# lovesh/bulletproofs-r1cs-gadgets

Hardware: AMD Instinct MI355X
Metric: R1CS proofs/sec (Poseidon VSMT-4 depth-32) (higher is better)
Workload: dtype int32; 1 GPU; gadget_vsmt_4 sparse-Merkle depth-32 membership (Poseidon 4:1 inverse S-box, 148 rounds); distinct_inputs_steps=9, batch_per_gpu=1024, global_batch=1024, n_multipliers=18656, padded_n=32768, constraints=43330, proof_bytes=1377, proofs_per_device_job=4096, device_jobs=3, jobs_in_flight=2, warmup_steps_run=5, ipa_unfold_rounds=4, table_window_bits=11, table_windows=23, table_format=1, table_bytes=197767468800

## Files before the change

bulletproofs-r1cs-gadgets_amd/csrc/api_prove.hpp:

```cpp
#pragma once
#include "ipa.hpp"
#include "host_chain.hpp"
struct bpr1cs_job {
    const bpr1cs_gens* g = nullptr;
    dev_stream_t st{}, st2{}, st3{}, st4{};
    std::vector<void*> deferred;
    PhaseTimer pt;
    MsmStats msm;
    uint32_t B = 0, m = 0;
    size_t plen = 0;
    uint8_t* h_proofs = nullptr;
    uint8_t* h_comms = nullptr;
    int* h_err = nullptr;
    uint32_t* h_chk = nullptr;
    strobe* h_tr = nullptr;
    bool counted = false;
    int slot = -1;
    IpaIO::TailKeep tail;
    dev_event_t ev_in{}, ev_rng{}, ev_wit{}, ev_done{}, ev_tail{};
    uint8_t* h_in = nullptr;
    size_t h_in_bytes = 0;
    uint8_t* h_V = nullptr;
    uint64_t* h_raw = nullptr;
    size_t h_raw_bytes = 0;
    strobe* h_tr0 = nullptr;
    bool host_chain = false;
    uint32_t Bh = 0;
    dev_event_t ev_head{};
};
struct HostStage {
    std::mutex mu;
    std::multimap<size_t, void*> cache;
    std::map<void*, size_t> live;
};
inline HostStage& host_stage() {
    static HostStage* h = new HostStage();
    return *h;
}
static void* host_stage_alloc(size_t n) {
    if (n == 0) n = 1;
#if defined(BPR1CS_HOSTSIM)
    return malloc(n);
#else
    HostStage& hs = host_stage();
    std::lock_guard<std::mutex> lk(hs.mu);
    auto it = hs.cache.lower_bound(n);
    void* p = nullptr;
    size_t sz = n;
    if (it != hs.cache.end() && it->first <= 2 * n + 4096) { p = it->second; sz = it->first; hs.cache.erase(it); }
    else HIPCHK(hipHostMalloc(&p, n, hipHostMallocDefault));
    hs.live[p] = sz;
    return p;
#endif
}
static void host_stage_free(void* p) {
#if defined(BPR1CS_HOSTSIM)
    free(p);
#else
    if (!p) return;
    HostStage& hs = host_stage();
    std::lock_guard<std::mutex> lk(hs.mu);
    auto it = hs.live.find(p);
    if (it == hs.live.end()) return;
    hs.cache.insert({it->second, p});
    hs.live.erase(it);
#endif
}
static bool dbg_jobs() {
    static const bool on = getenv("BPR1CS_DEBUG_JOBS") != nullptr;
    return on;
}
static double dbg_ms() {
    static const auto t0 = std::chrono::steady_clock::now();
    return std::chrono::duration<double, std::milli>(std::chrono::steady_clock::now() - t0).count();
}
#define DBG_JOB(...) do { if (dbg_jobs()) { fprintf(stderr, "bpr1cs[%9.2f ms] ", dbg_ms()); fprintf(stderr, __VA_ARGS__); fputc('\n', stderr); } } while (0)
static void host_wipe(void* p, size_t n) { explicit_bzero(p, n); }
static void job_wait(bpr1cs_job* job) {
    if (!job) return;
    if (job->ev_done) (void)dev_event_sync(job->ev_done);
#if !defined(BPR1CS_HOSTSIM)
    else if (job->st) (void)hipStreamSynchronize(job->st);
    if (job->st2) (void)hipStreamSynchronize(job->st2);
    if (job->st3) (void)hipStreamSynchronize(job->st3);
#endif
}
static void job_release(bpr1cs_job* job) {
    if (!job) return;
    job_wait(job);
#if !defined(BPR1CS_HOSTSIM)
    for (auto e : job->pt.ev) (void)hipEventDestroy(e);
    job->pt.ev.clear();
#endif
    dev_event_t* evs[6] = {&job->ev_in, &job->ev_rng, &job->ev_wit, &job->ev_done, &job->ev_tail, &job->ev_head};
    for (auto e : evs) dev_event_destroy(e);
    for (void* p : job->deferred) dev_free_now(p);
    job->deferred.clear();
    if (job->h_raw) host_wipe(job->h_raw, job->h_raw_bytes);
    if (job->h_in) host_wipe(job->h_in, job->h_in_bytes);
    if (job->h_tr0 && job->Bh) host_wipe(job->h_tr0, (size_t)job->Bh * sizeof(strobe));
    host_stage_free(job->h_in);
    host_stage_free(job->h_raw);
    host_stage_free(job->h_V);
    host_stage_free(job->h_tr0);
    host_stage_free(job->h_proofs);
    host_stage_free(job->h_comms);
    host_stage_free(job->h_err);
    host_stage_free(job->h_chk);
    host_stage_free(job->h_tr);
    if (job->counted) job->g->in_flight--;
    if (job->slot >= 0) job->g->busy_slots.fetch_and(~(1u << job->slot));
    delete job;
}

static TabCfg merged_tab_cfg(const bpr1cs_gens* g, uint32_t T3) {
#if defined(BPR1CS_HOSTSIM)
    const char* force = getenv("BPR1CS_TEST_NARROW_MERGED");
// ... 21 lines not shown
static void enqueue_witness_check(const bpr1cs_circuit* c, const sc* W, const sc* v_m, uint32_t* res, uint32_t B, dev_stream_t s) {
    {
        std::lock_guard<std::mutex> lk(c->mt_mu);
        if (!c->rows_uploaded) {
            ArenaScope persistent(nullptr);
            upload(c->row_off, c->h_row_off, s);
            upload(c->row_slot, c->h_row_slot, s);
            upload(c->row_coeff, c->h_row_coeff, s);
            upload(c->row_chunk, c->h_row_chunk, s);
            c->rows_uploaded = true;
        }
    }
    const uint32_t Bpad = (B + 63u) & ~63u;
    launch(B, K_check_init{res}, s);
    launch((uint64_t)((c->n + CHECK_GATES - 1) / CHECK_GATES) * Bpad, K_check_gates{W, res, B, Bpad, c->n}, s);
    const uint32_t nchunks = (uint32_t)c->h_row_chunk.size() - 1, per_launch = 0xffffffffu / Bpad;
    for (uint32_t c0 = 0; c0 < nchunks; c0 += per_launch)
        launch((uint64_t)std::min(per_launch, nchunks - c0) * Bpad,
               K_check_rows{c->row_chunk.p, c->row_off.p, c->row_slot.p, c->row_coeff.p, W, v_m, res, B, Bpad, 3 * c->n, c->m, c0}, s);
}

static int prove_job_begin(const bpr1cs_gens* g, const bpr1cs_circuit* c, const strobe* init, size_t n_init, bool want_tr,
                           const uint8_t* values, const uint8_t* v_blindings, const uint8_t* rng_seeds,
                           const uint8_t* wires, size_t batch, bpr1cs_job** job_out, const uint8_t* ext_draws = nullptr, int auto_share = 0) {
    if (!g || !c || !init || (!rng_seeds && !ext_draws) || !job_out || batch == 0 || (n_init != 1 && n_init != batch)) return BPR1CS_ERR_INVALID_ARGUMENT;
    if (ext_draws && n_init != batch) return BPR1CS_ERR_INVALID_ARGUMENT;
    if (c->m && (!values || !v_blindings)) return BPR1CS_ERR_INVALID_ARGUMENT;
    if (!have_device()) return BPR1CS_ERR_NO_DEVICE;
    if (g->cap < c->N) return BPR1CS_ERR_INVALID_GENERATORS_LENGTH;
    if (!wires && !c->has_program) return BPR1CS_ERR_MISSING_ASSIGNMENT;
    if (batch > (1u << 20) || ((uint64_t)4 * c->N + 3ull * c->n + c->m + 64) * batch > 0xffffffffull) return BPR1CS_ERR_INVALID_ARGUMENT;
    if (c->m && (!host_scalars_canonical(values, batch * c->m) || !host_scalars_canonical(v_blindings, batch * c->m))) return BPR1CS_ERR_INVALID_ARGUMENT;
    if (wires && !host_scalars_canonical(wires, batch * 3 * (size_t)c->n)) return BPR1CS_ERR_INVALID_ARGUMENT;
    bpr1cs_job* job = nullptr;
    struct Scope {
        std::vector<void*>* prev;
        explicit Scope(bpr1cs_job* j) : prev(dev_deferred_frees()) { dev_deferred_frees() = &j->deferred; }
        ~Scope() { dev_deferred_frees() = prev; }
    };
    uint32_t slot = 0;
    for (;;) {
        uint32_t busy = g->busy_slots.load();
        if ((busy & 3u) == 3u) return BPR1CS_ERR_INVALID_ARGUMENT;
        slot = (busy & 1u) ? 1u : 0u;
        if (g->busy_slots.compare_exchange_weak(busy, busy | (1u << slot))) break;
    }
    try {
// ... 60 lines not shown
        HIPCHK(hipGetLastError());
    } else
#endif
    launch((uint64_t)m * B, K_commit_v{g->tab.p, g->tc, v_raw.p, vbl_raw.p, Vcomp.p, B, m}, sl);
    DevBuf<strobe> tr(B);
    const bool shared = g->opts.shared_back.load() != 0;
    DevBuf<sc> blind((size_t)8 * B), W;
    DevBuf<uint64_t> rng_raw;
    const uint32_t draws = 2 * n + 7;
    const int o_hc = g->opts.host_chain.load();
    const bool ext = ext_draws != nullptr;
    const bool host_chain = !ext && (o_hc < 0 ? B <= 4u * host_cpu_budget() : B <= (uint32_t)o_hc);
    job->host_chain = host_chain;
    uint32_t Bh = 0;
    const unsigned chain_workers = host_cpu_budget() - 1;
#if !defined(BPR1CS_HOSTSIM)
    if (!ext && !host_chain && chain_workers > 0) {
        const int o_share = g->opts.host_chain_share.load();
        const int share = o_share >= 0 ? o_share : std::max(0, std::min(100, auto_share));
        Bh = (uint32_t)(((uint64_t)B * (uint32_t)share + 50) / 100);
    }
#endif
    job->Bh = Bh;
    {
        ArenaScope sh(shared ? &g->shared_front : &g->front[slot], shared);
        W.alloc((size_t)5 * n * B + 1);
        rng_raw.alloc((size_t)(draws + (host_chain || ext ? 1 : 0)) * B * 8);
    }
    sc* sL = W.p + (size_t)3 * n * B;
    sc* sR = W.p + (size_t)4 * n * B;
    pt.mark(sl);
    dev_event_create(&job->ev_in);
    dev_event_create(&job->ev_rng);
    dev_event_record(job->ev_in, sl);
    DevBuf<int> rng_err(1);
    dev_zero(rng_err.p, sizeof(int), sl);
    DevBuf<strobe> rng;
    HostChains chains;
    if (ext) {
        job->h_raw_bytes = (size_t)(draws + 1) * B * 64;
        job->h_raw = (uint64_t*)host_stage_alloc(job->h_raw_bytes);
        memcpy(job->h_raw, ext_draws, job->h_raw_bytes);
        dev_d2d(tr.p, d_init.p, (size_t)B * sizeof(strobe), sl);
        if (shared) dev_stream_wait(sl, g->rng_free_ev);
        dev_h2d_async(rng_raw.p, job->h_raw, job->h_raw_bytes, sl);
        if (shared) dev_stream_wait(sl, g->w_free_ev);
        launch((uint64_t)(draws + 1) * B, K_rng_reduce{rng_raw.p, blind.p, sL, sR, B, n, 1u}, sl);
        dev_zero(rng_raw.p, rng_raw.bytes(), sl);
        if (shared) dev_event_record(g->rng_free_ev, sl);
        dev_event_record(job->ev_rng, sl);
    } else if (host_chain) {
        job->h_V = (uint8_t*)host_stage_alloc((size_t)B * m * 32);
        if (m) dev_d2h_async(job->h_V, Vcomp.p, (size_t)B * m * 32, sl);
        job->h_raw_bytes = (size_t)(draws + 1) * B * 64;
        job->h_raw = (uint64_t*)host_stage_alloc(job->h_raw_bytes);
        job->h_tr0 = (strobe*)host_stage_alloc((size_t)B * sizeof(strobe));
    } else {
#if defined(BPR1CS_HOSTSIM)
        launch_transcript(B, K_transcript_init{d_init.p, init_stride, Vcomp.p, vbl_raw.p, d_seeds.p, tr.p, blind.p, sL, sR, nullptr, B, m, n}, sl);
#else
        rng.alloc(B);
        launch_transcript(B, K_transcript_init{d_init.p, init_stride, Vcomp.p, vbl_raw.p, d_seeds.p, tr.p, blind.p, sL, sR, rng.p, B, m, n}, sl);
        if (Bh) {
            job->h_tr0 = (strobe*)host_stage_alloc((size_t)Bh * sizeof(strobe));
            dev_d2h_async(job->h_tr0, rng.p, (size_t)Bh * sizeof(strobe), sl);
            dev_event_create(&job->ev_head);
            dev_event_record(job->ev_head, sl);
        }
        if (shared) dev_stream_wait(sl, g->rng_free_ev);
        if (Bh < B) {
            hipLaunchKernelGGL(k_rng_stream, dim3((B - Bh + 1) / 2), dim3(64), 0, sl, rng.p + Bh, rng_raw.p + (size_t)draws * Bh * 8, rng_err.p, B - Bh, draws);
            HIPCHK(hipGetLastError());
        }
        if (!Bh) {
            if (shared) dev_stream_wait(sl, g->w_free_ev);
            launch((uint64_t)draws * B, K_rng_reduce{rng_raw.p, blind.p, sL, sR, B, n, 0u}, sl);
            dev_zero(rng_raw.p, rng_raw.bytes(), sl);
            dev_zero(rng.p, rng.bytes(), sl);
            if (shared) dev_event_record(g->rng_free_ev, sl);
        }
#endif
        if (!Bh) dev_event_record(job->ev_rng, sl);
    }

    if (host_chain) {
        dev_sync(sl);
        DBG_JOB("begin: %u host chain(s) start", B);
        chains.start(init, n_init, job->h_V, v_blindings, rng_seeds, B, m, n, job->h_tr0, job->h_raw);
        if ((uint64_t)B * (draws + 1) <= 4096) chains.wait();
    }

    DevBuf<sc> px;
    struct { uint32_t* p; } chk{nullptr};
    if (o_check) {
        DevBuf<uint32_t>& blk = g->check_res[slot];
        if (blk.n < (size_t)4 * B) { ArenaScope persistent(nullptr); blk.alloc((size_t)4 * B); }
        chk.p = blk.p;
    }
    if (wires) {
        const dev_stream_t sw = job->st3;
        DevBuf<sc> raw((size_t)3 * n * B);
        static_assert(sizeof(sc) == 32, "a canonical scalar's 32 little-endian bytes are an sc as they are");
        if (raw.bytes()) dev_h2d(raw.p, wires, raw.bytes(), sw);
        if (shared) dev_stream_wait(sw, g->w_free_ev);
        launch((uint64_t)3 * n * B, K_load_wires_pm{raw.p, W.p, B, 3 * n}, sw);
// ... 15 lines not shown
            kw.px = px.p; kw.pzf = pzf.p; kw.px_stride = c->px_stride;
        }
#if defined(BPR1CS_HOSTSIM)
        (void)o_team;
        launch(B, kw, st);
        if (o_check) enqueue_witness_check(c, W.p, v_m.p, chk.p, B, st);
#else
        int T = o_team;
        if (c->n_perms && (uint32_t)T < c->macro_width + 2) T = 16;
        kw.prio = 2;
        uint32_t blocks = (uint32_t)(((uint64_t)B * T + 63) / 64);
        dev_stream_wait(job->st3, job->ev_in);
        if (shared) dev_stream_wait(job->st3, g->w_free_ev);
        if (T == 4) hipLaunchKernelGGL(HIP_KERNEL_NAME(k_witness_team<4>), dim3(blocks), dim3(64), 0, job->st3, kw);
        else if (T == 8) hipLaunchKernelGGL(HIP_KERNEL_NAME(k_witness_team<8>), dim3(blocks), dim3(64), 0, job->st3, kw);
        else hipLaunchKernelGGL(HIP_KERNEL_NAME(k_witness_team<16>), dim3(blocks), dim3(64), 0, job->st3, kw);
        HIPCHK(hipGetLastError());
        if (o_check) enqueue_witness_check(c, W.p, v_m.p, chk.p, B, job->st3);
        dev_event_create(&job->ev_wit);
        dev_event_record(job->ev_wit, job->st3);
        dev_stream_wait(st, job->ev_wit);
#endif
    }
    auto finish_split = [&]() {
        if (!Bh) return;
        const uint32_t Dc = 256, R = 4;
        const dev_stream_t su = job->st3;
        if (!dev_event_sync(job->ev_head)) throw DevError{BPR1CS_ERR_DEVICE};
        job->h_raw_bytes = (size_t)R * Dc * Bh * 64;
        job->h_raw = (uint64_t*)host_stage_alloc(job->h_raw_bytes);
        if (shared) dev_stream_wait(su, g->rng_free_ev);
        dev_event_t ev_slot[R] = {};
        for (uint32_t r = 0; r < R; r++) dev_event_create(&ev_slot[r]);
        struct Events { dev_event_t* e; uint32_t n; ~Events() { for (uint32_t r = 0; r < n; r++) dev_event_destroy(&e[r]); } } evs_guard{ev_slot, R};
        uint64_t* raw_h = rng_raw.p;
        DBG_JOB("begin: %u host chain(s) of %u streamed (%.4f us per permutation and worker)", Bh, B, host_chain_us_per_perm());
        double busy_us = 0;
        const bool ok = host_chains_stream(job->h_tr0, Bh, draws, Dc, R, job->h_raw, chain_workers,
            [&](uint32_t, uint32_t slot, uint32_t d0, uint32_t nd) {
                dev_h2d_async(raw_h + (size_t)d0 * Bh * 8, job->h_raw + (size_t)slot * Dc * Bh * 8, (size_t)nd * Bh * 64, su);
                dev_event_record(ev_slot[slot], su);
            },
            [&](uint32_t slot) { if (!dev_event_sync(ev_slot[slot])) throw DevError{BPR1CS_ERR_DEVICE}; }, chain8_select(), &busy_us);
        if (ok && busy_us > 0) host_chain_rate_cell().store(busy_us / ((double)Bh * draws));
        host_wipe(job->h_tr0, (size_t)Bh * sizeof(strobe));
        if (!ok) throw DevError{BPR1CS_ERR_INVALID_ARGUMENT};
        DBG_JOB("begin: host chain(s) hashed");
        dev_event_record(job->ev_head, su);
        dev_stream_wait(sl, job->ev_head);
        if (shared) dev_stream_wait(sl, g->w_free_ev);
        launch((uint64_t)draws * Bh, K_rng_reduce{raw_h, blind.p, sL, sR, B, n, 0u, Bh, 0u}, sl);
        if (Bh < B) launch((uint64_t)draws * (B - Bh), K_rng_reduce{raw_h + (size_t)draws * Bh * 8, blind.p, sL, sR, B, n, 0u, B - Bh, Bh}, sl);
        dev_zero(rng_raw.p, rng_raw.bytes(), sl);
        dev_zero(rng.p, rng.bytes(), sl);
        if (shared) dev_event_record(g->rng_free_ev, sl);
        dev_event_record(job->ev_rng, sl);
    };
    auto finish_host_chains = [&]() {
        finish_split();
        if (!host_chain) return;
        chains.wait();
        DBG_JOB("begin: host chain(s) done");
        dev_h2d_async(tr.p, job->h_tr0, (size_t)B * sizeof(strobe), sl);
        if (shared) dev_stream_wait(sl, g->rng_free_ev);
        dev_h2d_async(rng_raw.p, job->h_raw, job->h_raw_bytes, sl);
        if (shared) dev_stream_wait(sl, g->w_free_ev);
        launch((uint64_t)(draws + 1) * B, K_rng_reduce{rng_raw.p, blind.p, sL, sR, B, n, 1u}, sl);
        dev_zero(rng_raw.p, rng_raw.bytes(), sl);
        if (shared) dev_event_record(g->rng_free_ev, sl);
        dev_event_record(job->ev_rng, sl);
    };
    DBG_JOB("begin: front enqueued");
    DevBuf<uint8_t> AOS((size_t)3 * B * 32);
    DevBuf<sc> chal((size_t)CH_COUNT * B), txs((size_t)3 * B), uk((size_t)(lgN ? lgN : 1) * 2 * B);
    DevBuf<uint8_t> Tc((size_t)5 * B * 32), LR((size_t)(lgN ? lgN : 1) * 2 * B * 32);
    const size_t plen = bpr1cs_proof_len(c);
    job->plen = plen;
    DevBuf<uint8_t> d_out((size_t)B * plen);
    ArenaScope back_arena(shared ? &g->arena : &g->front[slot], shared);
    DevBuf<ge> partial, partialO;
    MsmPlan plan;
    {
// ... 28 lines not shown
                }
                mtab = mt->tab.p;
                mtc = mt->tc;
                ones_pt = mt->ones_pt.p;
            }
            const uint32_t nr = (uint32_t)c->h_rest.size();
            MsmSeg rG{aL, nr, 1, 1, 0, baseG, 1, c->rest.p, 0}, rH{aR, nr, 1, 1, 0, baseH, 1, c->rest.p, 0};
            MsmSeg mG{aL, T3, 1, 1, 0, 0, 1, c->trip.p, 1}, mH{aR, T3, 1, 1, 0, T3, 1, c->trip.p, 1};
            MsmPlan plan2;
            MsmSeg oRest{aO, nr, 1, 1, 0, baseG, MSM_MONT, c->rest.p, 0}, oOnes{aO, 2 * T3, 1, 1, 0, baseG, MSM_MINUS_ONE, c->ones.p, 0};
            MsmReq rq[4] = {{rG, rH, &partial, &plan, nullptr}, {mG, mH, &partial2, &plan2, mtab, 0, &mtc}, {oRest, none, &partialO, &planO, nullptr},
                            {oOnes, none, &partialO1, &planO1, nullptr, 256}};
            run_msm_multi(g, rq, 4, B, st, stats);
            finI.partial = partial.p;
            finI.nchunks = plan.nchunks;
            finI.partial_b = partial2.p;
            finI.nchunks_b = plan2.nchunks;
        } else {
            MsmReq rq[2] = {{seg(aL, baseG), seg(aR, baseH), &partial, &plan, nullptr}, {seg(aO, baseG), none, &partialO, &planO, nullptr}};
            run_msm_multi(g, rq, 2, B, st, stats, nullptr, ct);
            finI.partial = partial.p;
            finI.nchunks = plan.nchunks;
        }
        finish_host_chains();
        dev_stream_wait(st, job->ev_rng);
        pt.mark(st);
        if (ct) {
            DevBuf<ge> pbI, pbO, pbS;
            MsmPlan plI, plO, plS;
            auto bl = [&](uint32_t k) { return MsmSeg{blind.p + (size_t)k * B, 1, 1, 1, 0, 1, MSM_MONT}; };
            MsmReq rq[4] = {{seg(sL, baseG), seg(sR, baseH), &partialS, &planS, nullptr}, {bl(0), none, &pbI, &plI, nullptr},
                            {bl(1), none, &pbO, &plO, nullptr}, {bl(2), none, &pbS, &plS, nullptr}};
            run_msm_multi(g, rq, 4, B, st, stats, nullptr, true);
            finI.extra = nullptr; finI.partial_b = pbI.p; finI.nchunks_b = plI.nchunks;
            K_msm_finish finO{g->tab.p, g->tc, partialO.p, nullptr, nullptr, AOS.p + 1 * (size_t)B * 32, B, planO.nchunks, 1};
            finO.partial_b = pbO.p; finO.nchunks_b = plO.nchunks;
            K_msm_finish finS{g->tab.p, g->tc, partialS.p, nullptr, nullptr, AOS.p + 2 * (size_t)B * 32, B, planS.nchunks, 1};
            finS.partial_b = pbS.p; finS.nchunks_b = plS.nchunks;
            launch(B, finI, st);
            launch(B, finO, st);
            launch(B, finS, st);
        } else {
        K_msm_finish finO{g->tab.p, g->tc, partialO.p, blind.p + 1 * (size_t)B, nullptr, AOS.p + 1 * (size_t)B * 32, B, planO.nchunks, 1};
        if (ones_pt) { finO.shared_pt = ones_pt; finO.partial_b = partialO1.p; finO.nchunks_b = planO1.nchunks; }
        if (B <= SMALL_JOB_PROOFS) {
            run_msm(g, seg(sL, baseG), seg(sR, baseH), B, partialS, planS, st, stats);
            launch_finish_triple(finI, finO, K_msm_finish{g->tab.p, g->tc, partialS.p, blind.p + 2 * (size_t)B, nullptr, AOS.p + 2 * (size_t)B * 32, B, planS.nchunks, 1}, B, st);
        } else {
            launch_finish(finI, B, st);
            launch_finish(finO, B, st);
            run_msm(g, seg(sL, baseG), seg(sR, baseH), B, partial, plan, st, stats);
            launch_finish(K_msm_finish{g->tab.p, g->tc, partial.p, blind.p + 2 * (size_t)B, nullptr, AOS.p + 2 * (size_t)B * 32, B, plan.nchunks, 1}, B, st);
        }
        }
    }
    pt.mark(st);

    launch_transcript(B, K_transcript_A{tr.p, AOS.p, chal.p, B}, st);
    uint32_t maxe = std::max<uint32_t>(N, c->q + 1);
    uint32_t H = (maxe >> 8) + 1;
    DevBuf<sc> plo((size_t)3 * 256 * B), phi((size_t)3 * H * B);
    launch_pow_tables(K_pow_tables{chal.p, plo.p, phi.p, B, H}, B, st);
    const uint32_t r_eff = std::min<uint32_t>((uint32_t)o_unfold, lgN);
    const bool fvec = g->opts.factor_vectors.load() == 1;
    const uint32_t nfl = c->h_slot_chunk[3 * n + m];
    auto al = [](size_t x) { return (x + 255) & ~(size_t)255; };
    const size_t w_bytes = al(((size_t)(3 * n + m) * B + 1) * sizeof(sc)), p_bytes = al((size_t)(nfl ? nfl : 1) * B * sizeof(sc)),
                 v_bytes = al((size_t)N * B * sizeof(sc));
    const size_t vt_count = r_eff < lgN ? (size_t)VB_MULT * 4 * ((N >> r_eff) / 2 ? (N >> r_eff) / 2 : 1) * B : 0;
    const bool need_s = r_eff > 0 || (!fvec && lgN > 0);
    const size_t others = w_bytes + p_bytes + (fvec ? 2 * v_bytes : 0) + (need_s ? 2 * v_bytes : 0);
    DevBuf<uint8_t> shared_blk(std::max(others, vt_count * sizeof(ge_cached)));
    sc* wvec_p = (sc*)shared_blk.p;
    sc* fpart_p = (sc*)(shared_blk.p + w_bytes);
    uint8_t* nxt = shared_blk.p + w_bytes + p_bytes;
// ... 233 lines not shown
    J = std::min(J, grid_max);
    const size_t m = c->m, plen = bpr1cs_proof_len(c), wn = 3 * (size_t)c->n;
    struct Pending { bpr1cs_job* job; size_t first; };
    std::vector<Pending> fl;
    int rc = BPR1CS_OK;
    size_t ended = 0;
    auto finish_oldest = [&]() {
        Pending p = fl.front();
        fl.erase(fl.begin());
        ended += p.job->B;
        int e = prove_job_end(p.job, proofs_out + p.first * plen, commitments_out ? commitments_out + p.first * m * 32 : nullptr,
                              tr_out ? tr_out + p.first : nullptr, &acc);
        if (e != BPR1CS_OK && rc == BPR1CS_OK) rc = e;
    };
    size_t done = 0;
    bool retried = false;
    double prior_ms_per_proof = 0;
    {
        std::lock_guard<std::mutex> lk(c->mt_mu);
        auto it = c->mt.find(g);
        if (it != c->mt.end()) prior_ms_per_proof = it->second->msm_ms_per_proof;
    }
    auto auto_share = [&](size_t take) -> int {
        if (fl.empty() || ext_draws || g->opts.host_chain_share.load() >= 0) return 0;
        const uint32_t draws = 2 * c->n + 7;
        const size_t before = fl.back().job->B;
        const double per_proof = ended && acc.msm_ms > 0 ? acc.msm_ms / ended : prior_ms_per_proof;
        const double deadline_ms = per_proof > 0 ? per_proof * before : draws * 2.5e-3;
        return host_chain_share_auto(chain8_select() != chain8_advance_scalar, take, draws, host_cpu_budget() - 1, host_chain_us_per_perm(), deadline_ms);
    };
#if defined(BPR1CS_HOSTSIM)
    const char* inj = getenv("BPR1CS_TEST_FAIL_JOBS");
    int inject_oom = inj ? atoi(inj) : 0;
#else
    int inject_oom = 0;
#endif
    while (done < batch && rc == BPR1CS_OK) {
        const size_t rest = batch - done, take = std::min(J, rest);
        bpr1cs_job* job = nullptr;
        int e;
        if (inject_oom > 0) { inject_oom--; e = BPR1CS_ERR_OUT_OF_MEMORY; }
        else e = prove_job_begin(g, c, n_init == 1 ? init : init + done, n_init == 1 ? 1 : take, tr_out != nullptr,
                                 values ? values + done * m * 32 : nullptr, v_blindings ? v_blindings + done * m * 32 : nullptr,
                                 rng_seeds ? rng_seeds + done * 32 : nullptr, wires ? wires + done * wn * 32 : nullptr, take, &job,
                                 ext_draws ? ext_draws + done * (2 * (size_t)c->n + 8) * 64 : nullptr, auto_share(take));
        if (e == BPR1CS_ERR_OUT_OF_MEMORY && (take > 64 || !retried)) {
            while (!fl.empty()) finish_oldest();
            g->arena.release();
            g->front[0].release();
            g->front[1].release();
            g->shared_front.release();
            circuit_cache_purge();
#if !defined(BPR1CS_HOSTSIM)
            dev_pool().release_all();
#endif
            if (retried) {
                J = std::max<size_t>(64, std::min(J, take) / 2);
                if (automatic) g->sizing_epoch++;
            }
            retried = !retried;
            continue;
        }
        if (e != BPR1CS_OK) { rc = e; break; }
        retried = false;
        fl.push_back({job, done});
        done += take;
        if ((int)fl.size() >= depth) finish_oldest();
    }
// ... 69 lines not shown
```

bulletproofs-r1cs-gadgets_amd/csrc/host_chain.hpp:

```cpp
#pragma once
#include <thread>
#include <vector>
#include <atomic>
#include <algorithm>
#include <functional>
#include <mutex>
#include <condition_variable>
#include <chrono>
#include <stdio.h>
#include <stdlib.h>
#include <string.h>
#if defined(__linux__)
#include <sched.h>
#endif
#if defined(__x86_64__) && !defined(__HIP_DEVICE_COMPILE__)
#include <immintrin.h>
#endif
#include "merlin.hpp"

static unsigned host_cpu_budget() {
    static const unsigned cached = []() -> unsigned {
        unsigned n = std::thread::hardware_concurrency();
        if (n == 0) n = 1;
#if defined(__linux__)
// ... 96 lines not shown
#undef HC8_LD
#undef HC8_ST
#undef X3
#undef CHI
#undef ROL
}
#endif
typedef void (*chain8_fn)(Chain8&, unsigned, uint32_t, uint64_t*, size_t, size_t);
static chain8_fn chain8_select(bool allow_avx512 = true) {
#if defined(__x86_64__) && !defined(__HIP_DEVICE_COMPILE__)
    if (allow_avx512 && __builtin_cpu_supports("avx512f")) return chain8_advance_avx512;
#endif
    (void)allow_avx512;
    return chain8_advance_scalar;
}

static const unsigned HOST_SHARE_MIN_WORKERS = 2;
static int host_chain_share_auto(bool eight_way, uint64_t B, uint32_t draws, unsigned workers, double us_per_perm, double deadline_ms) {
    if (!eight_way || workers < HOST_SHARE_MIN_WORKERS || B == 0 || draws == 0 || !(us_per_perm > 0) || !(deadline_ms > 0)) return 0;
    const double whole_ms = (double)B * draws * us_per_perm / workers / 1e3;
    const double share = 100.0 * 0.75 * deadline_ms / whole_ms;
    return share >= 100.0 ? 100 : (int)share;
}
static std::atomic<double>& host_chain_rate_cell() {
    static std::atomic<double> cell{0.0};
    return cell;
}
static double host_chain_us_per_perm() {
    static const double calibrated = []() {
        Chain8 g;
        for (int k = 0; k < 25; k++)
            for (int p = 0; p < 8; p++) g.st[k][p] = 0x9e3779b97f4a7c15ull * (uint64_t)(25 * p + k + 1);
        std::vector<uint64_t> out((size_t)256 * 64);
        const chain8_fn fn = chain8_select();
        fn(g, 8, 16, out.data(), 8, 64);
        const auto t0 = std::chrono::steady_clock::now();
        fn(g, 8, 256, out.data(), 8, 64);
        const double us = std::chrono::duration<double, std::micro>(std::chrono::steady_clock::now() - t0).count();
        return 1.25 * us / (256.0 * 8);
    }();
    const double measured = host_chain_rate_cell().load();
    return measured > 0 ? measured : calibrated;
}

static bool host_chains_stream(const strobe* st, uint32_t P, uint32_t draws, uint32_t D, uint32_t R, uint64_t* ring, unsigned T,
                               const std::function<void(uint32_t, uint32_t, uint32_t, uint32_t)>& upload, const std::function<void(uint32_t)>& slot_free,
// ... 101 lines not shown
```

bulletproofs-r1cs-gadgets_amd/csrc/kernels.hpp:

```cpp
#pragma once
#include "fe.hpp"
#include "sc.hpp"
#include "ge.hpp"
#include "merlin.hpp"
#include "msm_trace.hpp"

struct TabCfg {
    uint32_t W, windows, entries, row, per_base;
    uint32_t stride;
    HD size_t base_bytes() const { return (size_t)per_base * stride; }
};
HD inline TabCfg tab_cfg(uint32_t W) {
    TabCfg t;
    t.W = W;
    t.windows = (252 + W) / W;
    t.entries = 1u << (W - 1);
    t.row = t.entries + 1;
    t.per_base = t.windows * t.row;
    t.stride = 128;
    return t;
}
HD inline int tab_digit(const sc& s, uint32_t k, int& carry, const TabCfg& tc) {
    uint32_t bit = k * tc.W, wi = bit >> 5, sh = bit & 31;
    uint64_t two = (uint64_t)s.v[wi] | ((wi + 1 < 8) ? ((uint64_t)s.v[wi + 1] << 32) : 0);
// ... 203 lines not shown
            uint8_t w[32];
            sc_store_raw(vbl_raw[(size_t)j * B + b], w);
            merlin_rng_rekey(r, "v_blinding", 10, w, 32);
        }
        merlin_rng_finalize(r, seeds + 32 * (size_t)b);
        blind[(size_t)0 * B + b] = merlin_rng_scalar(r);
        if (rng_out) {
            rng_out[b] = r;
            return;
        }
        for (int k = 1; k < 3; k++) blind[(size_t)k * B + b] = merlin_rng_scalar(r);
        for (uint32_t i = 0; i < n; i++) sL[(size_t)i * B + b] = merlin_rng_scalar(r);
        for (uint32_t i = 0; i < n; i++) sR[(size_t)i * B + b] = merlin_rng_scalar(r);
        for (int k = 3; k < 8; k++) blind[(size_t)k * B + b] = merlin_rng_scalar(r);
    }
};
struct K_rng_reduce {
    const uint64_t* raw;
    sc* blind;
    sc* sL;
    sc* sR;
    uint32_t B, n, lead;
    uint32_t Bc = 0, b0 = 0;
    HD void operator()(uint32_t g) const {
        uint32_t d, b;
        if (lead) {
            b = g / (2 * n + 8); d = g % (2 * n + 8);
        } else if (Bc) {
            d = g / Bc; b = b0 + g % Bc;
        } else {
            d = g / B; b = g % B;
        }
        sc x = sc_mont_from_wide_lanes(raw + (size_t)g * 8);
        if (lead) {
            if (d == 0) { blind[b] = x; return; }
            d -= 1;
        }
        if (d < 2) blind[(size_t)(1 + d) * B + b] = x;
        else if (d < 2 + n) sL[(size_t)(d - 2) * B + b] = x;
        else if (d < 2 + 2 * n) sR[(size_t)(d - 2 - n) * B + b] = x;
        else blind[(size_t)(3 + d - 2 - 2 * n) * B + b] = x;
    }
};

struct K_transcript_A {
    strobe* tr;
    const uint8_t* AOS;
    sc* chal;
// ... 1738 lines not shown
```

bulletproofs-r1cs-gadgets_amd/csrc/kernels_hip.hpp:

```cpp
#pragma once
#include <hip/hip_runtime.h>
#include "kernels.hpp"
#include "fe_wide.hpp"

struct fe_pow_wave {
    __device__ fe operator()(const fe& z) const { return fe_pow22523_wave(z); }
};
__device__ inline void ge_compress_wave(const ge& p, uint8_t* out) {
    uint8_t enc[32];
    ge_compress_t(p, enc, fe_pow_wave{});
    if ((threadIdx.x & 63u) == 0) {
#pragma unroll
        for (int i = 0; i < 32; i++) out[i] = enc[i];
    }
}

template <int T>
__device__ inline sc team_sum(sc acc) {
#pragma unroll
    for (int s = T / 2; s > 0; s >>= 1) {
        sc o;
#pragma unroll
        for (int k = 0; k < 8; k++) o.v[k] = (uint32_t)__shfl_xor((int)acc.v[k], s, T);
        acc = sc_add(acc, o);
// ... 419 lines not shown
    const uint32_t c = w * 64u + threadIdx.x;
    ge acc = c < f.nchunks ? f.chunk_sum(c, b) : ge_identity();
#pragma unroll 1
    for (int sft = 32; sft > 0; sft >>= 1) acc = ge_add_ge(acc, ge_shfl_xor(acc, sft));
    if (threadIdx.x == 0) f.partial[(size_t)w * f.B + b] = acc;
}

__global__ void __launch_bounds__(64) k_ge_reduce_wave(const ge* in_a, ge* out_a, const ge* in_b, ge* out_b, uint32_t B, uint32_t in_cnt, uint32_t groups) {
    const uint32_t per_req = groups * B;
    const uint32_t wg = blockIdx.x, r = wg / per_req, rest = wg % per_req, w = rest / B, b = rest % B;
    const ge* in = r ? in_b : in_a;
    ge* out = r ? out_b : out_a;
    const uint32_t c = w * 64u + threadIdx.x;
    ge acc = c < in_cnt ? in[(size_t)c * B + b] : ge_identity();
#pragma unroll 1
    for (int sft = 32; sft > 0; sft >>= 1) acc = ge_add_ge(acc, ge_shfl_xor(acc, sft));
    if (threadIdx.x == 0) out[(size_t)w * B + b] = acc;
}

#define K_XOR3(a, b, c) __builtin_amdgcn_bitop3_b32((a), (b), (c), 0x96)
#define K_CHI(a, b, c) __builtin_amdgcn_bitop3_b32((a), (b), (c), 0xd2)
__device__ inline void lds_order() { __syncthreads(); }
#define LDS_HANDOFF() do { __atomic_signal_fence(__ATOMIC_SEQ_CST); __builtin_amdgcn_wave_barrier(); __atomic_signal_fence(__ATOMIC_SEQ_CST); } while (0)
__global__ void __launch_bounds__(64) k_rng_stream(const strobe* rng_in, uint64_t* raw_out, int* err, uint32_t B, uint32_t draws) {
    __builtin_amdgcn_s_setprio(3);
    __shared__ uint64_t xch[2][32];
    __shared__ uint64_t colp[2][8];
    const uint32_t lane = threadIdx.x, i = lane & 31u, half = lane >> 5;
    uint32_t b = blockIdx.x * 2u + half;
    const bool valid = b < B;
    if (!valid) b = B - 1;
    const uint32_t j = i % 25u, x = j % 5u, y = j / 5u;
    uint64_t a = rng_in[b].st[j];
    if (rng_in[b].pos != 64 || rng_in[b].pos_begin != 0) {
        if (i == 0) atomicExch(err, 1);
        return;
    }
    const int ROT[25] = {0, 1, 62, 28, 27, 36, 44, 6, 55, 20, 3, 10, 43, 25, 39, 41, 45, 15, 21, 8, 18, 2, 61, 56, 14};
    const int rot = ROT[j];
    const bool rot_swap = rot >= 32 || rot == 0;
    const uint32_t rot_k = (32u - ((uint32_t)rot & 31u)) & 31u;
    const uint32_t iota_mask = j == 0 ? 0xffffffffu : 0u;
    const uint32_t xm = (x + 4u) % 5u, xp = (x + 1u) % 5u;
    const uint32_t s0 = (x + 3u * y) % 5u + 5u * x;
    const uint32_t x1 = (x + 1u) % 5u, x2 = (x + 2u) % 5u;
    const uint32_t s1 = (x1 + 3u * y) % 5u + 5u * x1, s2 = (x2 + 3u * y) % 5u + 5u * x2;
    uint64_t* A1 = xch[half];
// ... 10 lines not shown
        for (int r = 0; r < 24; r++) {
            if (real) __hip_atomic_fetch_xor(&C[x], a, __ATOMIC_RELAXED, __HIP_MEMORY_SCOPE_WORKGROUP);
            LDS_HANDOFF();
            uint64_t m = C[xm], p = C[xp];
            LDS_HANDOFF();
            if (y == 0u) C[x] = 0;
            uint32_t tl = K_XOR3(LO(a), LO(m), __builtin_amdgcn_alignbit(LO(p), HI(p), 31));
            uint32_t th = K_XOR3(HI(a), HI(m), __builtin_amdgcn_alignbit(HI(p), LO(p), 31));
            uint32_t ul = rot_swap ? th : tl, uh = rot_swap ? tl : th;
            uint32_t nl = __builtin_amdgcn_alignbit(ul, uh, rot_k), nh = __builtin_amdgcn_alignbit(uh, ul, rot_k);
            A1[i] = ((uint64_t)nh << 32) | nl;
            LDS_HANDOFF();
            uint64_t b0 = A1[s0], b1 = A1[s1], b2 = A1[s2];
            uint32_t cl = K_CHI(LO(b0), LO(b1), LO(b2)), ch = K_CHI(HI(b0), HI(b1), HI(b2));
            cl = __builtin_amdgcn_bitop3_b32(cl, (uint32_t)KECCAK_RC[r], iota_mask, 0x78);
            ch = __builtin_amdgcn_bitop3_b32(ch, (uint32_t)(KECCAK_RC[r] >> 32), iota_mask, 0x78);
            a = ((uint64_t)ch << 32) | cl;
            LDS_HANDOFF();
        }
        if (i < 8) {
            if (valid) raw_out[((size_t)d * B + b) * 8 + i] = a;
            a = 0;
        }
    }
#undef LO
#undef HI
}


__global__ void __launch_bounds__(256) k_probe_mad(uint32_t* out, uint32_t iters) {
    uint32_t t = threadIdx.x + blockIdx.x * 256u;
    int64_t a0 = t * 3 + 1, a1 = t * 5 + 1, a2 = t * 7 + 2, a3 = t * 11 + 3, a4 = t + 9, a5 = t + 17, a6 = t ^ 0x55, a7 = t ^ 0x99;
    int32_t x = (int32_t)(t | 1), y = (int32_t)((t * 2654435761u) | 1);
    for (uint32_t i = 0; i < iters; i++) {
        asm volatile("v_mad_i64_i32 %0, vcc, %8, %9, %0\n\tv_mad_i64_i32 %1, vcc, %8, %9, %1\n\tv_mad_i64_i32 %2, vcc, %8, %9, %2\n\tv_mad_i64_i32 %3, vcc, %8, %9, %3\n\t"
                     "v_mad_i64_i32 %4, vcc, %8, %9, %4\n\tv_mad_i64_i32 %5, vcc, %8, %9, %5\n\tv_mad_i64_i32 %6, vcc, %8, %9, %6\n\tv_mad_i64_i32 %7, vcc, %8, %9, %7"
                     : "+v"(a0), "+v"(a1), "+v"(a2), "+v"(a3), "+v"(a4), "+v"(a5), "+v"(a6), "+v"(a7)
                     : "v"(x), "v"(y)
                     : "vcc");
    }
    out[t] = (uint32_t)(a0 ^ a1 ^ a2 ^ a3 ^ a4 ^ a5 ^ a6 ^ a7);
}
__global__ void __launch_bounds__(256) k_probe_madd(uint32_t* out, uint32_t iters) {
    uint32_t t = threadIdx.x + blockIdx.x * 256u;
    ge p = ge_basepoint();
    ge_niels q = ge_table_niels_identity();
// ... 100 lines not shown
```

bulletproofs-r1cs-gadgets_amd/csrc/msm_run.hpp:

```cpp
#pragma once
#include "api_common.hpp"
struct PhaseTimer {
#if defined(BPR1CS_HOSTSIM)
    void mark(dev_stream_t) {}
    void finish(float*) {}
#else
    std::vector<hipEvent_t> ev;
    void mark(dev_stream_t s) {
        hipEvent_t e;
        HIPCHK(hipEventCreate(&e));
        HIPCHK(hipEventRecord(e, s));
        ev.push_back(e);
    }
    void finish(float* out) {
        if (ev.size() < 2) return;
        HIPCHK(hipEventSynchronize(ev.back()));
        HIPCHK(hipEventElapsedTime(&out[0], ev.front(), ev.back()));
        for (size_t i = 1; i < ev.size() && i < 6; i++) HIPCHK(hipEventElapsedTime(&out[i], ev[i - 1], ev[i]));
        for (auto e : ev) (void)hipEventDestroy(e);
        ev.clear();
    }
#endif
};

// ... 312 lines not shown
        terms += (uint64_t)total * B;
        adds += (uint64_t)total * B * (ct ? g->tc_ct.windows : q.tc ? q.tc->windows : g->tc.windows);
        wg += nchunks * nbk;
        if (ct) L.job[r] = MsmJob{{q.s0, q.s1}, g->tab_ct.p, g->tc_ct, lay[r].raw, q.plan->chunk, nchunks, 0};
        else L.job[r] = MsmJob{{q.s0, q.s1}, q.table ? q.table : g->tab.p, q.tc ? *q.tc : g->tc, lay[r].raw, q.plan->chunk, nchunks, 0};
        L.wg_end[r] = wg;
    }
    if (ct) launch_msm_ct_kernel(L, st, stats, terms, adds);
    else launch_msm_kernel(g, L, st, stats, terms, adds);
    for (uint32_t r = 0; r < nreq; r++) {
        if (lay[r].l1) launch((uint64_t)lay[r].l1 * B, K_ge_reduce{lay[r].raw, lay[r].p1, B, lay[r].nchunks, MSM_REDUCE_GROUP}, st);
        if (lay[r].l2) launch((uint64_t)lay[r].l2 * B, K_ge_reduce{lay[r].p1, lay[r].p2, B, lay[r].l1, MSM_REDUCE_GROUP}, st);
    }
}
static void run_commit_ct(const bpr1cs_gens* g, const sc* s0, const sc* s1, uint32_t form, uint32_t count, uint8_t* out, uint32_t B, uint32_t m,
                          dev_stream_t st, MsmStats* stats) {
    if (!count) return;
    DevBuf<ge> partial;
    MsmPlan plan;
    MsmReq q{MsmSeg{s0, 1, 1, 1, 0, 0, form}, MsmSeg{s1, 1, 1, 1, 0, 1, form}, &partial, &plan, nullptr};
    run_msm_multi(g, &q, 1, count, st, stats, nullptr, true);
    launch(count, K_ct_finish{partial.p, plan.nchunks, count, out, B, m}, st);
}
static void run_msm(const bpr1cs_gens* g, MsmSeg s0, MsmSeg s1, uint32_t B, DevBuf<ge>& partial, MsmPlan& plan, dev_stream_t st,
                    MsmStats* stats, const uint8_t* table = nullptr) {
    MsmReq q{s0, s1, &partial, &plan, table};
    run_msm_multi(g, &q, 1, B, st, stats);
}

static void run_flatten(const bpr1cs_circuit* c, uint32_t nslots, const sc* plo, const sc* phi, sc* wvec, uint32_t B, uint32_t H, dev_stream_t st,
                        sc* part_buf = nullptr ) {
    uint32_t nch = c->h_slot_chunk[nslots];
    DevBuf<sc> part;
    if (!part_buf) { part.alloc((size_t)(nch ? nch : 1) * B); part_buf = part.p; }
    launch((uint64_t)nch * B, K_flatten_chunks{c->chunk_lo.p, c->ent_row.p, c->ent_coeff.p, plo, phi, part_buf, B, H}, st);
    launch((uint64_t)nslots * B, K_flatten{c->slot_chunk.p, part_buf, wvec, B, 3 * c->n}, st);
}

#if defined(BPR1CS_HOSTSIM)
extern "C" void bpr1cs_sim_msm_trace(int mode, uint64_t* out) {
    MsmTrace& t = msm_trace();
    if (out) {
        for (uint32_t k = 0; k < MSM_TR_KINDS; k++) { out[k] = t.count[k]; out[MSM_TR_KINDS + k] = t.hash[k]; }
        out[2 * MSM_TR_KINDS] = t.ct_launches;
        out[2 * MSM_TR_KINDS + 1] = t.fixed2_launches;
    }
// ... 5 lines not shown
```

Measured before the change: 2988 proofs/s.

## Split RNG draws in two halves and start sL MSM early on first job

For the first job of a call, the device RNG stream kernel now generates the first half of the draws, saves the strobe state, and then generates the rest. The sL blinding half is reduced first so the sL·G MSM can start on the main stream while the remaining draws and the host chains finish. The sR·H MSM then runs separately and its partials are merged in the finish kernel. A cold-start host-chain share heuristic based on CU count is also added, so the first job can offload some chains to the CPU without any prior timing history. Splitting the one combined MSM into two launches adds launch overhead and extra partial buffers.

```diff
diff --git a/bulletproofs-r1cs-gadgets_amd/csrc/api_prove.hpp b/bulletproofs-r1cs-gadgets_amd/csrc/api_prove.hpp
--- a/bulletproofs-r1cs-gadgets_amd/csrc/api_prove.hpp
+++ b/bulletproofs-r1cs-gadgets_amd/csrc/api_prove.hpp
@@ -27,6 +27,8 @@
     bool host_chain = false;
     uint32_t Bh = 0;
     dev_event_t ev_head{};
+    dev_event_t ev_rng_half{}, ev_rng_half_h{};
+    dev_event_t ev_rng_red{};
 };
 struct HostStage {
     std::mutex mu;
@@ -66,6 +68,15 @@
     hs.live.erase(it);
 #endif
 }
+static uint32_t dev_cu_count() {
+#if defined(BPR1CS_HOSTSIM)
+    return 256;
+#else
+    int dev = 0, cus = 0;
+    if (hipGetDevice(&dev) != hipSuccess || hipDeviceGetAttribute(&cus, hipDeviceAttributeMultiprocessorCount, dev) != hipSuccess) return 0;
+    return cus > 0 ? (uint32_t)cus : 0u;
+#endif
+}
 static bool dbg_jobs() {
     static const bool on = getenv("BPR1CS_DEBUG_JOBS") != nullptr;
     return on;
@@ -92,7 +103,8 @@
     for (auto e : job->pt.ev) (void)hipEventDestroy(e);
     job->pt.ev.clear();
 #endif
-    dev_event_t* evs[6] = {&job->ev_in, &job->ev_rng, &job->ev_wit, &job->ev_done, &job->ev_tail, &job->ev_head};
+    dev_event_t* evs[9] = {&job->ev_in, &job->ev_rng, &job->ev_wit, &job->ev_done, &job->ev_tail, &job->ev_head, &job->ev_rng_half, &job->ev_rng_half_h,
+                           &job->ev_rng_red};
     for (auto e : evs) dev_event_destroy(e);
     for (void* p : job->deferred) dev_free_now(p);
     job->deferred.clear();
@@ -160,7 +172,8 @@
 
 static int prove_job_begin(const bpr1cs_gens* g, const bpr1cs_circuit* c, const strobe* init, size_t n_init, bool want_tr,
                            const uint8_t* values, const uint8_t* v_blindings, const uint8_t* rng_seeds,
-                           const uint8_t* wires, size_t batch, bpr1cs_job** job_out, const uint8_t* ext_draws = nullptr, int auto_share = 0) {
+                           const uint8_t* wires, size_t batch, bpr1cs_job** job_out, const uint8_t* ext_draws = nullptr, int auto_share = 0,
+                           bool first_of_call = false) {
     if (!g || !c || !init || (!rng_seeds && !ext_draws) || !job_out || batch == 0 || (n_init != 1 && n_init != batch)) return BPR1CS_ERR_INVALID_ARGUMENT;
     if (ext_draws && n_init != batch) return BPR1CS_ERR_INVALID_ARGUMENT;
     if (c->m && (!values || !v_blindings)) return BPR1CS_ERR_INVALID_ARGUMENT;
@@ -267,6 +280,13 @@
     }
 #endif
     job->Bh = Bh;
+#if defined(BPR1CS_HOSTSIM)
+    const bool two_sum = false;
+    (void)first_of_call;
+#else
+    const bool two_sum = first_of_call && !ext && !host_chain && n > 0 && B > SMALL_JOB_PROOFS && !g->ct();
+#endif
+    const uint32_t d_half = n + 2;
     {
         ArenaScope sh(shared ? &g->shared_front : &g->front[slot], shared);
         W.alloc((size_t)5 * n * B + 1);
@@ -313,11 +333,20 @@
             dev_event_record(job->ev_head, sl);
         }
         if (shared) dev_stream_wait(sl, g->rng_free_ev);
-        if (Bh < B) {
-            hipLaunchKernelGGL(k_rng_stream, dim3((B - Bh + 1) / 2), dim3(64), 0, sl, rng.p + Bh, rng_raw.p + (size_t)draws * Bh * 8, rng_err.p, B - Bh, draws);
+        if (Bh < B && two_sum) {
+            const uint32_t Bd = B - Bh;
+            uint64_t* raw_d = rng_raw.p + (size_t)draws * Bh * 8;
+            hipLaunchKernelGGL(k_rng_stream, dim3((Bd + 1) / 2), dim3(64), 0, sl, rng.p + Bh, raw_d, rng_err.p, Bd, d_half, rng.p + Bh);
             HIPCHK(hipGetLastError());
-        }
-        if (!Bh) {
+            dev_event_create(&job->ev_rng_half);
+            dev_event_record(job->ev_rng_half, sl);
+            hipLaunchKernelGGL(k_rng_stream, dim3((Bd + 1) / 2), dim3(64), 0, sl, rng.p + Bh, raw_d + (size_t)d_half * Bd * 8, rng_err.p, Bd, draws - d_half, (strobe*)nullptr);
+            HIPCHK(hipGetLastError());
+        } else if (Bh < B) {
+            hipLaunchKernelGGL(k_rng_stream, dim3((B - Bh + 1) / 2), dim3(64), 0, sl, rng.p + Bh, rng_raw.p + (size_t)draws * Bh * 8, rng_err.p, B - Bh, draws, (strobe*)nullptr);
+            HIPCHK(hipGetLastError());
+        }
+        if (!Bh && !two_sum) {
             if (shared) dev_stream_wait(sl, g->w_free_ev);
             launch((uint64_t)draws * B, K_rng_reduce{rng_raw.p, blind.p, sL, sR, B, n, 0u}, sl);
             dev_zero(rng_raw.p, rng_raw.bytes(), sl);
@@ -325,7 +354,7 @@
             if (shared) dev_event_record(g->rng_free_ev, sl);
         }
 #endif
-        if (!Bh) dev_event_record(job->ev_rng, sl);
+        if (!Bh && !two_sum) dev_event_record(job->ev_rng, sl);
     }
 
     if (host_chain) {
@@ -387,8 +416,19 @@
         dev_stream_wait(st, job->ev_wit);
 #endif
     }
-    auto finish_split = [&]() {
-        if (!Bh) return;
+    auto finish_split = [&](const std::function<void()>& at_half) {
+        if (!Bh) {
+            if (!at_half) return;
+            at_half();
+            if (shared) dev_stream_wait(sl, g->w_free_ev);
+            launch((uint64_t)(draws - d_half) * B, K_rng_reduce{rng_raw.p, blind.p, sL, sR, B, n, 0u, 0u, 0u, d_half}, sl);
+            if (job->ev_rng_red) dev_stream_wait(sl, job->ev_rng_red);
+            dev_zero(rng_raw.p, rng_raw.bytes(), sl);
+            dev_zero(rng.p, rng.bytes(), sl);
+            if (shared) dev_event_record(g->rng_free_ev, sl);
+            dev_event_record(job->ev_rng, sl);
+            return;
+        }
         const uint32_t Dc = 256, R = 4;
         const dev_stream_t su = job->st3;
         if (!dev_event_sync(job->ev_head)) throw DevError{BPR1CS_ERR_DEVICE};
@@ -405,6 +445,13 @@
             [&](uint32_t, uint32_t slot, uint32_t d0, uint32_t nd) {
                 dev_h2d_async(raw_h + (size_t)d0 * Bh * 8, job->h_raw + (size_t)slot * Dc * Bh * 8, (size_t)nd * Bh * 64, su);
                 dev_event_record(ev_slot[slot], su);
+                if (two_sum && d0 <= d_half - 1 && d_half - 1 < d0 + nd) {
+                    if (shared) dev_stream_wait(su, g->w_free_ev);
+                    launch((uint64_t)d_half * Bh, K_rng_reduce{raw_h, blind.p, sL, sR, B, n, 0u, Bh, 0u, 0u}, su);
+                    dev_event_create(&job->ev_rng_half_h);
+                    dev_event_record(job->ev_rng_half_h, su);
+                    if (at_half) at_half();
+                }
             },
             [&](uint32_t slot) { if (!dev_event_sync(ev_slot[slot])) throw DevError{BPR1CS_ERR_DEVICE}; }, chain8_select(), &busy_us);
         if (ok && busy_us > 0) host_chain_rate_cell().store(busy_us / ((double)Bh * draws));
@@ -414,15 +461,17 @@
         dev_event_record(job->ev_head, su);
         dev_stream_wait(sl, job->ev_head);
         if (shared) dev_stream_wait(sl, g->w_free_ev);
-        launch((uint64_t)draws * Bh, K_rng_reduce{raw_h, blind.p, sL, sR, B, n, 0u, Bh, 0u}, sl);
-        if (Bh < B) launch((uint64_t)draws * (B - Bh), K_rng_reduce{raw_h + (size_t)draws * Bh * 8, blind.p, sL, sR, B, n, 0u, B - Bh, Bh}, sl);
+        const uint32_t r0 = two_sum ? d_half : 0u;
+        launch((uint64_t)(draws - r0) * Bh, K_rng_reduce{raw_h, blind.p, sL, sR, B, n, 0u, Bh, 0u, r0}, sl);
+        if (Bh < B) launch((uint64_t)(draws - r0) * (B - Bh), K_rng_reduce{raw_h + (size_t)draws * Bh * 8, blind.p, sL, sR, B, n, 0u, B - Bh, Bh, r0}, sl);
+        if (job->ev_rng_red) dev_stream_wait(sl, job->ev_rng_red);
         dev_zero(rng_raw.p, rng_raw.bytes(), sl);
         dev_zero(rng.p, rng.bytes(), sl);
         if (shared) dev_event_record(g->rng_free_ev, sl);
         dev_event_record(job->ev_rng, sl);
     };
-    auto finish_host_chains = [&]() {
-        finish_split();
+    auto finish_host_chains = [&](const std::function<void()>& at_half = nullptr) {
+        finish_split(at_half);
         if (!host_chain) return;
         chains.wait();
         DBG_JOB("begin: host chain(s) done");
@@ -497,7 +546,23 @@
             finI.partial = partial.p;
             finI.nchunks = plan.nchunks;
         }
-        finish_host_chains();
+        bool half_summed = false;
+        auto sum_first_half = [&]() {
+            if (half_summed) return;
+            half_summed = true;
+            if (job->ev_rng_half) {
+                dev_stream_wait(st, job->ev_rng_half);
+                if (shared) dev_stream_wait(st, g->w_free_ev);
+                launch((uint64_t)d_half * (B - Bh), K_rng_reduce{rng_raw.p + (size_t)draws * Bh * 8, blind.p, sL, sR, B, n, 0u, Bh ? B - Bh : 0u, Bh, 0u}, st);
+                dev_event_create(&job->ev_rng_red);
+                dev_event_record(job->ev_rng_red, st);
+            }
+            if (job->ev_rng_half_h) dev_stream_wait(st, job->ev_rng_half_h);
+            ArenaScope own(nullptr);
+            run_msm(g, seg(sL, baseG), none, B, partialS, planS, st, stats);
+            if (stats && stats->launches) stats->launches--;
+        };
+        finish_host_chains(two_sum ? std::function<void()>(sum_first_half) : std::function<void()>());
         dev_stream_wait(st, job->ev_rng);
         pt.mark(st);
         if (ct) {
@@ -524,8 +589,15 @@
         } else {
             launch_finish(finI, B, st);
             launch_finish(finO, B, st);
-            run_msm(g, seg(sL, baseG), seg(sR, baseH), B, partial, plan, st, stats);
-            launch_finish(K_msm_finish{g->tab.p, g->tc, partial.p, blind.p + 2 * (size_t)B, nullptr, AOS.p + 2 * (size_t)B * 32, B, plan.nchunks, 1}, B, st);
+            K_msm_finish finS{g->tab.p, g->tc, nullptr, blind.p + 2 * (size_t)B, nullptr, AOS.p + 2 * (size_t)B * 32, B, 0, 1};
+            if (two_sum) {
+                const size_t need = msm_partial_need(g, 2 * n, B);
+                if (partial.n < need) partial.alloc(need);
+                run_msm(g, seg(sR, baseH), none, B, partial, plan, st, stats);
+                finS.partial_b = partialS.p; finS.nchunks_b = planS.nchunks;
+            } else run_msm(g, seg(sL, baseG), seg(sR, baseH), B, partial, plan, st, stats);
+            finS.partial = partial.p; finS.nchunks = plan.nchunks;
+            launch_finish(finS, B, st);
         }
         }
     }
@@ -805,8 +877,13 @@
         if (it != c->mt.end()) prior_ms_per_proof = it->second->msm_ms_per_proof;
     }
     auto auto_share = [&](size_t take) -> int {
-        if (fl.empty() || ext_draws || g->opts.host_chain_share.load() >= 0) return 0;
+        if (ext_draws || g->opts.host_chain_share.load() >= 0) return 0;
         const uint32_t draws = 2 * c->n + 7;
+        if (fl.empty()) {
+            const unsigned workers = host_cpu_budget() - 1;
+            const double us = std::max(host_chain_us_per_perm(), workers * HOST_CHAIN_STREAM_US_PER_PERM);
+            return host_chain_share_first(chain8_select() != chain8_advance_scalar, take, draws, workers, us, 2u * 4u * dev_cu_count(), DEV_CHAIN_US_PER_PERM);
+        }
         const size_t before = fl.back().job->B;
         const double per_proof = ended && acc.msm_ms > 0 ? acc.msm_ms / ended : prior_ms_per_proof;
         const double deadline_ms = per_proof > 0 ? per_proof * before : draws * 2.5e-3;
@@ -826,7 +903,7 @@
         else e = prove_job_begin(g, c, n_init == 1 ? init : init + done, n_init == 1 ? 1 : take, tr_out != nullptr,
                                  values ? values + done * m * 32 : nullptr, v_blindings ? v_blindings + done * m * 32 : nullptr,
                                  rng_seeds ? rng_seeds + done * 32 : nullptr, wires ? wires + done * wn * 32 : nullptr, take, &job,
-                                 ext_draws ? ext_draws + done * (2 * (size_t)c->n + 8) * 64 : nullptr, auto_share(take));
+                                 ext_draws ? ext_draws + done * (2 * (size_t)c->n + 8) * 64 : nullptr, auto_share(take), fl.empty());
         if (e == BPR1CS_ERR_OUT_OF_MEMORY && (take > 64 || !retried)) {
             while (!fl.empty()) finish_oldest();
             g->arena.release();
diff --git a/bulletproofs-r1cs-gadgets_amd/csrc/host_chain.hpp b/bulletproofs-r1cs-gadgets_amd/csrc/host_chain.hpp
--- a/bulletproofs-r1cs-gadgets_amd/csrc/host_chain.hpp
+++ b/bulletproofs-r1cs-gadgets_amd/csrc/host_chain.hpp
@@ -142,6 +142,22 @@
     const double share = 100.0 * 0.75 * deadline_ms / whole_ms;
     return share >= 100.0 ? 100 : (int)share;
 }
+static const double DEV_CHAIN_US_PER_PERM = 2.5;
+static const double HOST_SHARE_FIRST_MIN_SAVED_US = 2000.0;
+static const double HOST_CHAIN_STREAM_US_PER_PERM = 0.0027;
+static int host_chain_share_first(bool eight_way, uint64_t B, uint32_t draws, unsigned workers, double us_per_perm, uint32_t dev_cap,
+                                  double dev_us_per_perm) {
+    if (!eight_way || workers < HOST_SHARE_MIN_WORKERS || B == 0 || draws == 0 || !(us_per_perm > 0) || !(dev_us_per_perm > 0) || dev_cap == 0) return 0;
+    if (B <= dev_cap) return 0;
+    const double dev_rate = dev_us_per_perm / dev_cap, host_rate = us_per_perm / workers;
+    const uint64_t balance = (uint64_t)((double)B * dev_rate / (dev_rate + host_rate));
+    const uint64_t Bh = std::min<uint64_t>(balance, B - dev_cap);
+    const double t_all = (double)draws * dev_rate * (double)B;
+    const double t_dev = (double)draws * dev_rate * (double)(B - Bh), t_host = (double)Bh * draws * host_rate;
+    const double saved = t_all - std::max(t_dev, t_host);
+    if (saved < 0.1 * t_all || saved < HOST_SHARE_FIRST_MIN_SAVED_US) return 0;
+    return (int)((100 * Bh + B / 2) / B);
+}
 static std::atomic<double>& host_chain_rate_cell() {
     static std::atomic<double> cell{0.0};
     return cell;
diff --git a/bulletproofs-r1cs-gadgets_amd/csrc/kernels.hpp b/bulletproofs-r1cs-gadgets_amd/csrc/kernels.hpp
--- a/bulletproofs-r1cs-gadgets_amd/csrc/kernels.hpp
+++ b/bulletproofs-r1cs-gadgets_amd/csrc/kernels.hpp
@@ -249,8 +249,10 @@
     sc* sR;
     uint32_t B, n, lead;
     uint32_t Bc = 0, b0 = 0;
+    uint32_t d0 = 0;
     HD void operator()(uint32_t g) const {
         uint32_t d, b;
+        if (!lead) g += d0 * (Bc ? Bc : B);
         if (lead) {
             b = g / (2 * n + 8); d = g % (2 * n + 8);
         } else if (Bc) {
diff --git a/bulletproofs-r1cs-gadgets_amd/csrc/kernels_hip.hpp b/bulletproofs-r1cs-gadgets_amd/csrc/kernels_hip.hpp
--- a/bulletproofs-r1cs-gadgets_amd/csrc/kernels_hip.hpp
+++ b/bulletproofs-r1cs-gadgets_amd/csrc/kernels_hip.hpp
@@ -465,7 +465,7 @@
 #define K_CHI(a, b, c) __builtin_amdgcn_bitop3_b32((a), (b), (c), 0xd2)
 __device__ inline void lds_order() { __syncthreads(); }
 #define LDS_HANDOFF() do { __atomic_signal_fence(__ATOMIC_SEQ_CST); __builtin_amdgcn_wave_barrier(); __atomic_signal_fence(__ATOMIC_SEQ_CST); } while (0)
-__global__ void __launch_bounds__(64) k_rng_stream(const strobe* rng_in, uint64_t* raw_out, int* err, uint32_t B, uint32_t draws) {
+__global__ void __launch_bounds__(64) k_rng_stream(const strobe* rng_in, uint64_t* raw_out, int* err, uint32_t B, uint32_t draws, strobe* rng_out) {
     __builtin_amdgcn_s_setprio(3);
     __shared__ uint64_t xch[2][32];
     __shared__ uint64_t colp[2][8];
@@ -522,6 +522,10 @@
             if (valid) raw_out[((size_t)d * B + b) * 8 + i] = a;
             a = 0;
         }
+    }
+    if (rng_out && valid) {
+        if (real) rng_out[b].st[j] = a;
+        if (i == 0) { const uint32_t f = rng_in[b].cur_flags; rng_out[b].pos = 64; rng_out[b].pos_begin = 0; rng_out[b].cur_flags = f; }
     }
 #undef LO
 #undef HI
diff --git a/bulletproofs-r1cs-gadgets_amd/csrc/msm_run.hpp b/bulletproofs-r1cs-gadgets_amd/csrc/msm_run.hpp
--- a/bulletproofs-r1cs-gadgets_amd/csrc/msm_run.hpp
+++ b/bulletproofs-r1cs-gadgets_amd/csrc/msm_run.hpp
@@ -358,6 +358,13 @@
     run_msm_multi(g, &q, 1, count, st, stats, nullptr, true);
     launch(count, K_ct_finish{partial.p, plan.nchunks, count, out, B, m}, st);
 }
+static size_t msm_partial_need(const bpr1cs_gens* g, uint32_t total, uint32_t B) {
+    uint32_t chunk, nchunks = pick_chunks(total, B, 1u << g->opts.msm_threads_log2.load(), chunk);
+    if (chunk < 8 && total >= 8) nchunks = (total + 7) / 8;
+    const uint32_t l1 = nchunks > MSM_REDUCE_GROUP ? (nchunks + MSM_REDUCE_GROUP - 1) / MSM_REDUCE_GROUP : 0;
+    const uint32_t l2 = l1 > MSM_REDUCE_GROUP ? (l1 + MSM_REDUCE_GROUP - 1) / MSM_REDUCE_GROUP : 0;
+    return ((size_t)nchunks + l1 + l2) * B;
+}
 static void run_msm(const bpr1cs_gens* g, MsmSeg s0, MsmSeg s1, uint32_t B, DevBuf<ge>& partial, MsmPlan& plan, dev_stream_t st,
                     MsmStats* stats, const uint8_t* table = nullptr) {
     MsmReq q{s0, s1, &partial, &plan, table};
```

After: 3041 proofs/s, median of 6. 1.02x the previous value.
